# 619862306/CODON

Hardware: AMD Instinct MI355X
Metric: HR depth maps/sec (fwd) (higher is better)
Workload: dtype f32

## Files before the change

codon_amd/csrc/conv_wgrad_f32.hip:

```cpp

#include "codon_common.h"
#include "kernels.h"

namespace codon {

struct WgradParams {
  const float* x;
  const float* gy;
  float* ws;
  int H, W, cin, cout;
  long x_img, g_img, x_base, g_base;
  int tiles_x, band_tiles_y, nbands;
  int nsplit;
};

template <int KS, int CO_T, int CI_T>
__global__ __launch_bounds__(256, 2) void conv_wgrad_f32_kernel(const WgradParams p) {
  constexpr int PAD = KS / 2;
  constexpr int TW = 32, TH = 4;
  constexpr int XR = TH + KS - 1, XQ = TW + KS - 1;
  constexpr int XPL = (XR * XQ) | 1;
  constexpr int GPL = (TH * TW) | 1;
  constexpr int NCI = CI_T * 32, NCO = CO_T * 32;
  constexpr int XS = NCI * XPL, GS = NCO * GPL;
  constexpr int TAPS = KS * KS;
  constexpr int NT = CO_T * CI_T * TAPS;
  constexpr int TPW = (NT + 3) / 4;
  constexpr int XE = (NCI * XR * XQ + 255) / 256;
  constexpr int GE = (NCO * TH * TW) / 256;

  __shared__ float lds[XS + GS];
  float* const xs = lds;
  float* const gs = lds + XS;

  const int tid = threadIdx.x, lane = tid & 63, wave = tid >> 6;
  const int l31 = lane & 31, half = lane >> 5;
  const int H = p.H, W = p.W;
  const long HW = (long)H * W;

  const int nci_t = p.cin / NCI;
  const int cot = blockIdx.x / nci_t, cit = blockIdx.x % nci_t;
  const int split = blockIdx.y;
  const int b = split / p.nbands, band = split % p.nbands;
  const int ty_begin = band * p.band_tiles_y;
  const int tiles_y = (H + TH - 1) / TH;
  const int ty_end = min(ty_begin + p.band_tiles_y, tiles_y);

  const float* __restrict__ xg = p.x + b * p.x_img + p.x_base + (long)cit * NCI * HW;
  const float* __restrict__ gg = p.gy + b * p.g_img + p.g_base + (long)cot * NCO * HW;

  int a_off[TPW], b_off[TPW];
#pragma unroll
  for (int j = 0; j < TPW; ++j) {
    int t = wave + 4 * j;
    if (t >= NT) t = NT - 1;
    const int tap = t % TAPS;
    const int cc = t / TAPS;
    const int ci_t = cc % CI_T, co_t = cc / CI_T;
    const int dy = tap / KS, dx = tap % KS;
    a_off[j] = (co_t * 32 + l31) * GPL + half;
    b_off[j] = (ci_t * 32 + l31) * XPL + dy * XQ + dx + half;
  }

  f32x16 acc[TPW];
#pragma unroll
  for (int j = 0; j < TPW; ++j)
#pragma unroll
    for (int r = 0; r < 16; ++r) acc[j][r] = 0.f;

#pragma unroll 1
  for (int ty = ty_begin; ty < ty_end; ++ty) {
#pragma unroll 1
    for (int tx = 0; tx < p.tiles_x; ++tx) {
      const int tx0 = tx * TW, ty0 = ty * TH;
      __syncthreads();
#pragma unroll 6
      for (int k = 0; k < XE; ++k) {
        const int e = tid + k * 256;
        const int c = e / (XR * XQ);
        const int rem = e - c * (XR * XQ);
        const int r = rem / XQ, q = rem - r * XQ;
        const int gy_ = ty0 + r - PAD, gx_ = tx0 + q - PAD;
        if (e < NCI * XR * XQ) {
          const bool ok = gy_ >= 0 && gy_ < H && gx_ >= 0 && gx_ < W;
          const float v = xg[ok ? c * HW + (long)gy_ * W + gx_ : 0];
          xs[c * XPL + rem] = ok ? v : 0.f;
        }
      }
#pragma unroll 8
      for (int k = 0; k < GE; ++k) {
        const int e = tid + k * 256;
        const int c = e / (TH * TW);
        const int rem = e - c * (TH * TW);
        const int r = rem / TW, q = rem - r * TW;
        const int gy_ = ty0 + r, gx_ = tx0 + q;
        const bool ok = gy_ < H && gx_ < W;
        const float v = gg[ok ? c * HW + (long)gy_ * W + gx_ : 0];
        gs[c * GPL + rem] = ok ? v : 0.f;
      }
      __syncthreads();
#pragma unroll 1
      for (int r = 0; r < TH; ++r) {
#pragma unroll 4
        for (int q = 0; q < TW; q += 2) {
          const int po = r * TW + q, xo = r * XQ + q;
#pragma unroll
          for (int j = 0; j < TPW; ++j) {
            const float a = gs[a_off[j] + po];
            const float bv = xs[b_off[j] + xo];
            acc[j] = __builtin_amdgcn_mfma_f32_32x32x2f32(a, bv, acc[j], 0, 0, 0);
          }
        }
      }
    }
  }

  float* __restrict__ wsp = p.ws + (long)split * TAPS * p.cout * p.cin;
#pragma unroll
  for (int j = 0; j < TPW; ++j) {
    const int t = wave + 4 * j;
    if (t < NT) {
      const int tap = t % TAPS;
      const int cc = t / TAPS;
      const int ci_t = cc % CI_T, co_t = cc / CI_T;
      const int ci = cit * NCI + ci_t * 32 + l31;
#pragma unroll
      for (int r = 0; r < 16; ++r) {
        const int co = cot * NCO + co_t * 32 + (r & 3) + 8 * (r >> 2) + 4 * half;
        wsp[((long)tap * p.cout + co) * p.cin + ci] = acc[j][r];
      }
    }
  }
}

__global__ __launch_bounds__(256) void wgrad_reduce_kernel(const float* __restrict__ ws, float* __restrict__ dw,
                                                           int cout, int cin, int taps, int nsplit, int accumulate) {
  const long n = (long)cout * cin * taps;
  const long i = (blockIdx.x * 256L + threadIdx.x) * 4;
  if (i >= n) return;
  const int ci = (int)(i % cin);
  const long t = i / cin;
  const int co = (int)(t % cout);
  const int tap = (int)(t / cout);
  float4 s = make_float4(0.f, 0.f, 0.f, 0.f);
  int k = 0;
  for (; k + 8 <= nsplit; k += 8) {
    float4 v[8];
#pragma unroll
    for (int j = 0; j < 8; ++j) v[j] = *reinterpret_cast<const float4*>(ws + (long)(k + j) * n + i);
#pragma unroll
    for (int j = 0; j < 8; ++j) { s.x += v[j].x; s.y += v[j].y; s.z += v[j].z; s.w += v[j].w; }
  }
  for (; k < nsplit; ++k) {
    const float4 v = *reinterpret_cast<const float4*>(ws + (long)k * n + i);
    s.x += v.x; s.y += v.y; s.z += v.z; s.w += v.w;
  }
  float* o = dw + ((long)co * cin + ci) * taps + tap;
  const float r[4] = {s.x, s.y, s.z, s.w};
#pragma unroll
  for (int j = 0; j < 4; ++j) o[(long)j * taps] = accumulate ? o[(long)j * taps] + r[j] : r[j];
}

int launch_wgrad_reduce(const float* ws, float* dw, int cout, int cin, int taps, int nsplit, int accumulate,
                        hipStream_t stream) {
  const long n = (long)cout * cin * taps;
  if (cin % 4 != 0 || ((uintptr_t)ws % 16) != 0) {
    set_error("wgrad_reduce: cin %d not a multiple of 4 or workspace not 16-byte aligned", cin);
    return CODON_ERR_BAD_ARG;
  }
  hipLaunchKernelGGL(wgrad_reduce_kernel, dim3((unsigned)((n / 4 + 255) / 256)), dim3(256), 0, stream, ws, dw, cout, cin,
                     taps, nsplit, accumulate);
  return check_launch("wgrad_reduce_kernel");
}

struct WgradPlan {
  int co_t, ci_t, nbands, band_tiles_y, nsplit, nchan_blocks;
  bool t16;
};

static bool wgrad_plan(const codon_conv_desc* d, WgradPlan* pl) {
  const int k = d->ksize, ci = d->cin, co = d->cout;
  if (k == 5 && ((ci == 128 && co == 128) || (ci == 64 && co == 64))) { pl->co_t = 1; pl->ci_t = 1; }
  else if (k == 3 && ((ci == 64 || ci == 128) && co == 64)) { pl->co_t = 2; pl->ci_t = 1; }
  else if (k == 1 && ci == 128 && co == 64) { pl->co_t = 2; pl->ci_t = 2; }
  else return false;
  pl->nchan_blocks = (co / (32 * pl->co_t)) * (ci / (32 * pl->ci_t));
  pl->t16 = conv_wgrad_f32_t16_shape(d);
  const int plan_blocks = pl->t16 ? (co / 64) * (ci / (k == 1 ? 128 : 32)) : pl->nchan_blocks;
  const int target = pl->t16 ? 256 : 1024;
  const int tiles_y = (d->height + 3) / 4;
  const int want = wgrad_band_count(target, plan_blocks, d->batch, tiles_y);
  pl->band_tiles_y = (tiles_y + want - 1) / want;
  pl->nbands = (tiles_y + pl->band_tiles_y - 1) / pl->band_tiles_y;
  pl->nsplit = d->batch * pl->nbands;
  return true;
}

size_t conv_wgrad_workspace_bytes(const codon_conv_desc* d) {
  WgradPlan pl;
  if (!wgrad_plan(d, &pl)) return 0;
  return (size_t)pl.nsplit * d->cout * d->cin * d->ksize * d->ksize * sizeof(float);
}

template <int KS, int CO_T, int CI_T>
static void launch_wgrad(const WgradParams& p, int nchan_blocks, hipStream_t stream) {
  hipLaunchKernelGGL((conv_wgrad_f32_kernel<KS, CO_T, CI_T>), dim3(nchan_blocks, p.nsplit), dim3(256), 0, stream, p);
}

int conv2d_wgrad_f32(const codon_conv_desc* d, const float* x, const float* gy, float* dw, float* workspace,
                     size_t ws_bytes, int accumulate, hipStream_t stream) {
  WgradPlan pl;
  if (!wgrad_plan(d, &pl)) {
    set_error("conv2d_wgrad: no f32 kernel for k=%d cin=%d cout=%d", d->ksize, d->cin, d->cout);
    return CODON_ERR_UNSUPPORTED;
  }
  CODON_REQUIRE(ws_bytes >= conv_wgrad_workspace_bytes(d), CODON_ERR_BAD_ARG,
                "conv2d_wgrad: workspace %zu B < required %zu B", ws_bytes, conv_wgrad_workspace_bytes(d));
  CODON_REQUIRE(pl.nsplit <= 65535, CODON_ERR_UNSUPPORTED, "conv2d_wgrad: %d splits > 65535", pl.nsplit);
  if (pl.t16 && conv_wgrad_f32_t16_supported(d, x, gy)) {
    const int st = launch_wgrad_f32_t16(d, x, gy, workspace, pl.nbands, pl.nsplit, stream);
    if (st != CODON_OK || accumulate == CODON_WGRAD_DEFER) return st;
    return launch_wgrad_reduce(workspace, dw, d->cout, d->cin, d->ksize * d->ksize, pl.nsplit, accumulate, stream);
  }
  WgradParams p = wgrad_fill<WgradParams>(d, x, gy, workspace, 1, pl.nbands, pl.nsplit);
  p.band_tiles_y = pl.band_tiles_y;
  if (d->ksize == 5) launch_wgrad<5, 1, 1>(p, pl.nchan_blocks, stream);
  else if (d->ksize == 3) launch_wgrad<3, 2, 1>(p, pl.nchan_blocks, stream);
  else launch_wgrad<1, 2, 2>(p, pl.nchan_blocks, stream);
  int st = check_launch("conv_wgrad_f32_kernel");
  if (st != CODON_OK || accumulate == CODON_WGRAD_DEFER) return st;
  return launch_wgrad_reduce(workspace, dw, d->cout, d->cin, d->ksize * d->ksize, pl.nsplit, accumulate, stream);
}

}
```

codon_amd/csrc/conv_wgrad_f32_t16.hip:

```cpp

#include <type_traits>

#include "codon_common.h"
#include "kernels.h"

namespace codon {

typedef unsigned t16_u32x4 __attribute__((ext_vector_type(4)));
typedef unsigned t16_u32x2 __attribute__((ext_vector_type(2)));

typedef const volatile __attribute__((address_space(3))) float* lds_rf;

template <int N, class F, int I = 0>
__device__ __forceinline__ void t16_static_for(F&& f) {
  if constexpr (I < N) {
    f(std::integral_constant<int, I>{});
    t16_static_for<N, F, I + 1>(static_cast<F&&>(f));
  }
}

struct WgradT16Params {
  const float* x;
  const float* gy;
  float* ws;
  int H, W, cin, cout;
  long x_img, g_img, x_base, g_base;
  int tiles_x, nbands, nsplit;
};

template <int KS>
__global__ __launch_bounds__(512, 2) void conv_wgrad_f32_t16_kernel(const WgradT16Params p) {
  constexpr int PAD = KS / 2, TAPS = KS * KS;
  constexpr int NCIT = KS == 1 ? 4 : 1;
  constexpr int NCI = 32 * NCIT;
  constexpr int NACC = TAPS * NCIT;
  constexpr int TW = 32, TH = KS == 1 ? 2 : 4;
  constexpr int XL = KS == 1 ? 0 : 4;
  constexpr int XC = TW + 2 * XL, XR = TH + KS - 1;
  constexpr int XPL = ((XR * XC + 29) / 32) * 32 + 2;
  constexpr int GPL = TH * TW + 2;
  static_assert(XPL >= XR * XC && XPL % 32 == 2 && GPL % 32 == 2, "plane strides");
  constexpr int XW = NCI * XPL, GW = 64 * GPL;
  constexpr int NXC = NCI * XR * (XC / 4), NGC = 64 * TH * (TW / 4);
  constexpr int NT = 512;
  constexpr int XE = (NXC + NT - 1) / NT, GE = NGC / NT;
  static_assert(NGC % NT == 0, "gy tile is a whole number of staging rounds");
  constexpr unsigned OOB = 0xFFFFFFF0u;

  __shared__ __attribute__((aligned(16))) float lds[2 * (XW + GW)];

  const int tid = threadIdx.x, lane = tid & 63, wave = tid >> 6;
  const int l15 = lane & 15, kq = lane >> 4;
  const int H = p.H, W = p.W;
  const long HW = (long)H * W;
  const unsigned HW4 = 4u * (unsigned)H * (unsigned)W;

  const int nci_b = p.cin / NCI;
  const unsigned vb_ = xcd_remap(blockIdx.y * gridDim.x + blockIdx.x, gridDim.x * gridDim.y);
  const int bx_ = (int)(vb_ % gridDim.x), by_ = (int)(vb_ / gridDim.x);
  const int cob = bx_ / nci_b, cib = bx_ % nci_b;
  const int split = by_;
  const int b = split / p.nbands, band = split % p.nbands;
  const int tiles_y = (H + TH - 1) / TH;
  const int ty_begin = (int)((long)band * tiles_y / p.nbands);
  const int ty_end = (int)((long)(band + 1) * tiles_y / p.nbands);
  const int ntile = (ty_end - ty_begin) * p.tiles_x;

  const float* const xg = p.x + b * p.x_img + p.x_base + (long)cib * NCI * HW;
  const float* const gg = p.gy + b * p.g_img + p.g_base + (long)cob * 64 * HW;

  unsigned xrel[XE], grel[GE];
  int xrc[XE], grc[GE];
  int xlds[XE], glds[GE];
#pragma unroll
  for (int k = 0; k < XE; ++k) {
    const int e = tid + k * NT;
    const int ch = e % (XC / 4), r = (e / (XC / 4)) % XR, c = e / ((XC / 4) * XR);
    const bool in = (NXC % NT == 0) || e < NXC;
    xrel[k] = (unsigned)c * HW4 + 4u * (unsigned)(r * W + ch * 4);
    xrc[k] = in ? ((r << 8) | ch) : -1;
    xlds[k] = in ? c * XPL + r * XC + ch * 4 : 0;
  }
#pragma unroll
  for (int k = 0; k < GE; ++k) {
    const int e = tid + k * NT;
    const int ch = e % (TW / 4), r = (e / (TW / 4)) % TH, c = e / ((TW / 4) * TH);
    grel[k] = (unsigned)c * HW4 + 4u * (unsigned)(r * W + ch * 4);
    grc[k] = (r << 8) | ch;
    glds[k] = c * GPL + r * TW + ch * 4;
  }

  const int co16 = wave & 3, ci16 = wave >> 2;
  const int a_lane = (co16 * 16 + l15) * GPL + kq;
  const int b_lane = (ci16 * 16 * NCIT + l15) * XPL + kq + (XL - PAD);

  f32x4 acc[NACC];
#pragma unroll
  for (int j = 0; j < NACC; ++j)
#pragma unroll
    for (int r = 0; r < 4; ++r) acc[j][r] = 0.f;

  t16_u32x4 xv[XE], gv[GE];
  auto load_tile = [&](int t) {
    const int ty = ty_begin + t / p.tiles_x, tx = t % p.tiles_x;
    const int tx0 = tx * TW, ty0 = ty * TH;
    const __amdgpu_buffer_rsrc_t xr = __builtin_amdgcn_make_buffer_rsrc(
        (void*)(xg + ((long)(ty0 - PAD) * W + (tx0 - XL))), 0, (int)OOB, 0x00020000);
    const __amdgpu_buffer_rsrc_t gr = __builtin_amdgcn_make_buffer_rsrc(
        (void*)(gg + ((long)ty0 * W + tx0)), 0, (int)OOB, 0x00020000);
#pragma unroll
    for (int k = 0; k < XE; ++k) {
      const int gy_ = ty0 - PAD + (xrc[k] >> 8), gx_ = tx0 - XL + 4 * (xrc[k] & 255);
      const bool ok = xrc[k] >= 0 && gy_ >= 0 && gy_ < H && gx_ >= 0 && gx_ < W;
      const auto v = __builtin_amdgcn_raw_buffer_load_b128(xr, ok ? xrel[k] : OOB, 0, 0);
      xv[k] = *reinterpret_cast<const t16_u32x4*>(&v);
    }
#pragma unroll
    for (int k = 0; k < GE; ++k) {
      const int gy_ = ty0 + (grc[k] >> 8), gx_ = tx0 + 4 * (grc[k] & 255);
      const bool ok = gy_ < H && gx_ < W;
      const auto v = __builtin_amdgcn_raw_buffer_load_b128(gr, ok ? grel[k] : OOB, 0, 0);
      gv[k] = *reinterpret_cast<const t16_u32x4*>(&v);
    }
  };
  auto store_tile = [&](int buf) {
    float* xs = lds + buf * (XW + GW);
    float* gs = xs + XW;
#pragma unroll
    for (int k = 0; k < XE; ++k)
      if ((NXC % NT == 0) || tid + k * NT < NXC) {
        *reinterpret_cast<t16_u32x2*>(xs + xlds[k]) = t16_u32x2{xv[k][0], xv[k][1]};
        *reinterpret_cast<t16_u32x2*>(xs + xlds[k] + 2) = t16_u32x2{xv[k][2], xv[k][3]};
      }
#pragma unroll
    for (int k = 0; k < GE; ++k) {
      *reinterpret_cast<t16_u32x2*>(gs + glds[k]) = t16_u32x2{gv[k][0], gv[k][1]};
      *reinterpret_cast<t16_u32x2*>(gs + glds[k] + 2) = t16_u32x2{gv[k][2], gv[k][3]};
    }
  };

  if (ntile > 0) {
    load_tile(0);
    store_tile(0);
  }
  __syncthreads();

#pragma unroll 1
  for (int t = 0; t < ntile; ++t) {
    const bool has_next = t + 1 < ntile;
    if (has_next) load_tile(t + 1);

    const float* xs = lds + (t & 1) * (XW + GW);
    const float* gs = xs + XW;
    const lds_rf ap = (lds_rf)(gs + a_lane);
    const lds_rf bp = (lds_rf)(xs + b_lane);
    float a[2], bv[2][NACC];
#define T16_FETCH(set_, r_, q_)                                                           \
    {                                                                                     \
      a[set_] = ap[(r_) * TW + (q_)];                                                     \
      _Pragma("unroll") for (int ct = 0; ct < NCIT; ++ct)                                 \
        _Pragma("unroll") for (int dy = 0; dy < KS; ++dy)                                 \
          _Pragma("unroll") for (int dx = 0; dx < KS; ++dx)                               \
            bv[set_][ct * TAPS + dy * KS + dx] = bp[ct * 16 * XPL + ((r_) + dy) * XC + (q_) + dx]; \
    }
    T16_FETCH(0, 0, 0)
    t16_static_for<TH * (TW / 4)>([&](auto sc) {
      constexpr int s_ = decltype(sc)::value;
      constexpr int cur = s_ & 1;
      if constexpr (s_ + 1 < TH * (TW / 4)) T16_FETCH(cur ^ 1, (s_ + 1) / (TW / 4), ((s_ + 1) % (TW / 4)) * 4)
      __builtin_amdgcn_sched_barrier(0);
#pragma unroll
      for (int j = 0; j < NACC; ++j) acc[j] = __builtin_amdgcn_mfma_f32_16x16x4f32(a[cur], bv[cur][j], acc[j], 0, 0, 0);
      __builtin_amdgcn_sched_barrier(0);
    });
#undef T16_FETCH
    if (has_next) store_tile((t + 1) & 1);
    __syncthreads();
  }

  float* __restrict__ wsp = p.ws + (long)split * TAPS * p.cout * p.cin;
#pragma unroll
  for (int ct = 0; ct < NCIT; ++ct) {
    const int ci = cib * NCI + (ci16 * NCIT + ct) * 16 + l15;
#pragma unroll
    for (int tap = 0; tap < TAPS; ++tap)
#pragma unroll
      for (int r = 0; r < 4; ++r) {
        const int co = cob * 64 + co16 * 16 + 4 * kq + r;
        wsp[((long)tap * p.cout + co) * p.cin + ci] = acc[ct * TAPS + tap][r];
      }
  }
}

bool conv_wgrad_f32_t16_shape(const codon_conv_desc* d) {
  if (d->ksize == 1 && d->cin % 128 != 0) return false;
  return (d->ksize == 1 || d->ksize == 3 || d->ksize == 5) && d->width % 4 == 0 && d->cout % 64 == 0 && d->cin % 32 == 0 &&
         (long)d->height * d->width * 4 * 128 < 0xFFFFFFF0L;
}

bool conv_wgrad_f32_t16_supported(const codon_conv_desc* d, const void* x, const void* gy) {
  if (!conv_wgrad_f32_t16_shape(d)) return false;
  const long HW = (long)d->height * d->width;
  const uintptr_t xa = reinterpret_cast<uintptr_t>(x) + 4 * (uintptr_t)(d->x_coff * HW);
  const uintptr_t ga = reinterpret_cast<uintptr_t>(gy) + 4 * (uintptr_t)(d->y_coff * HW);
  return (xa % 16) == 0 && (ga % 16) == 0 && ((d->x_ctotal * HW * 4) % 16) == 0 && ((d->y_ctotal * HW * 4) % 16) == 0;
}

int launch_wgrad_f32_t16(const codon_conv_desc* d, const float* x, const float* gy, float* workspace, int nbands,
                         int nsplit, hipStream_t stream) {
  const WgradT16Params p = wgrad_fill<WgradT16Params>(d, x, gy, workspace, 1, nbands, nsplit);
  const dim3 grid((d->cout / 64) * (d->cin / (d->ksize == 1 ? 128 : 32)), nsplit);
  if (d->ksize == 5) hipLaunchKernelGGL(conv_wgrad_f32_t16_kernel<5>, grid, dim3(512), 0, stream, p);
  else if (d->ksize == 3) hipLaunchKernelGGL(conv_wgrad_f32_t16_kernel<3>, grid, dim3(512), 0, stream, p);
  else hipLaunchKernelGGL(conv_wgrad_f32_t16_kernel<1>, grid, dim3(512), 0, stream, p);
  return check_launch("conv_wgrad_f32_t16_kernel");
}

}
```

Measured before the change: 32.27.

## Stage wgrad tiles with direct buffer-to-LDS loads interleaved into MFMA loop

Replaces the register-staged global load + LDS store of the next x/gy tile with per-dword buffer_load ... lds instructions. Their issue is spread across the first half of the MFMA K-loop, so copying the next tile overlaps compute without holding it in VGPRs. It adds an interior-tile fast path that skips per-element bounds checks and uses per-plane buffer resources. It also drops the width%4 and 16-byte alignment requirements, widening the t16 path to more shapes, but k=1 with unaligned width is routed back to the old kernel. The tradeoff is narrower 4-byte loads instead of 128-bit loads, plus a waitcnt/barrier at each tile end.

After: 32.21. About the same (-0.2%).

```diff
diff --git a/codon_amd/csrc/conv_wgrad_f32.hip b/codon_amd/csrc/conv_wgrad_f32.hip
--- a/codon_amd/csrc/conv_wgrad_f32.hip
+++ b/codon_amd/csrc/conv_wgrad_f32.hip
@@ -186,8 +186,9 @@
   else return false;
   pl->nchan_blocks = (co / (32 * pl->co_t)) * (ci / (32 * pl->ci_t));
   pl->t16 = conv_wgrad_f32_t16_shape(d);
-  const int plan_blocks = pl->t16 ? (co / 64) * (ci / (k == 1 ? 128 : 32)) : pl->nchan_blocks;
-  const int target = pl->t16 ? 256 : 1024;
+  const bool plan_t16 = pl->t16 && d->width % 4 == 0;
+  const int plan_blocks = plan_t16 ? (co / 64) * (ci / (k == 1 ? 128 : 32)) : pl->nchan_blocks;
+  const int target = plan_t16 ? 256 : 1024;
   const int tiles_y = (d->height + 3) / 4;
   const int want = wgrad_band_count(target, plan_blocks, d->batch, tiles_y);
   pl->band_tiles_y = (tiles_y + want - 1) / want;
@@ -217,7 +218,8 @@
   CODON_REQUIRE(ws_bytes >= conv_wgrad_workspace_bytes(d), CODON_ERR_BAD_ARG,
                 "conv2d_wgrad: workspace %zu B < required %zu B", ws_bytes, conv_wgrad_workspace_bytes(d));
   CODON_REQUIRE(pl.nsplit <= 65535, CODON_ERR_UNSUPPORTED, "conv2d_wgrad: %d splits > 65535", pl.nsplit);
-  if (pl.t16 && conv_wgrad_f32_t16_supported(d, x, gy)) {
+  const bool k1_recorded = d->ksize == 1 && d->width % 4 != 0;
+  if (pl.t16 && !k1_recorded && conv_wgrad_f32_t16_supported(d, x, gy)) {
     const int st = launch_wgrad_f32_t16(d, x, gy, workspace, pl.nbands, pl.nsplit, stream);
     if (st != CODON_OK || accumulate == CODON_WGRAD_DEFER) return st;
     return launch_wgrad_reduce(workspace, dw, d->cout, d->cin, d->ksize * d->ksize, pl.nsplit, accumulate, stream);
diff --git a/codon_amd/csrc/conv_wgrad_f32_t16.hip b/codon_amd/csrc/conv_wgrad_f32_t16.hip
--- a/codon_amd/csrc/conv_wgrad_f32_t16.hip
+++ b/codon_amd/csrc/conv_wgrad_f32_t16.hip
@@ -41,15 +41,24 @@
   constexpr int GPL = TH * TW + 2;
   static_assert(XPL >= XR * XC && XPL % 32 == 2 && GPL % 32 == 2, "plane strides");
   constexpr int XW = NCI * XPL, GW = 64 * GPL;
-  constexpr int NXC = NCI * XR * (XC / 4), NGC = 64 * TH * (TW / 4);
-  constexpr int NT = 512;
-  constexpr int XE = (NXC + NT - 1) / NT, GE = NGC / NT;
-  static_assert(NGC % NT == 0, "gy tile is a whole number of staging rounds");
+  constexpr int NWV = 8;
+  constexpr int XPLANE = XR * XC, GPLANE = TH * TW;
+  constexpr int XJ = (XPLANE + 63) / 64, GJ = GPLANE / 64;
+  static_assert(GPLANE % 64 == 0 && XJ * 64 <= XPL && GJ * 64 <= GPL, "a piece stays inside its padded plane");
+  constexpr int XPW = NCI / NWV, GPW = 64 / NWV;
+  static_assert(NCI % NWV == 0, "x planes are dealt evenly over the waves");
+  constexpr int NPX = XPW * XJ, NPIECE = NPX + GPW * GJ;
+  constexpr int NSTEP = TH * (TW / 4);
+  constexpr int PPS = KS == 1 ? 8 : 2;
+  static_assert(PPS * (NSTEP / 2 + 2) >= NPIECE, "the tile's pieces are all issued by the middle of the K loop");
   constexpr unsigned OOB = 0xFFFFFFF0u;
+  constexpr int RSRC_FLAGS = 0x00020000;
+  typedef __attribute__((address_space(3))) void lds_void;
 
   __shared__ __attribute__((aligned(16))) float lds[2 * (XW + GW)];
 
-  const int tid = threadIdx.x, lane = tid & 63, wave = tid >> 6;
+  const int tid = threadIdx.x, lane = tid & 63;
+  const int wave = __builtin_amdgcn_readfirstlane(tid >> 6);
   const int l15 = lane & 15, kq = lane >> 4;
   const int H = p.H, W = p.W;
   const long HW = (long)H * W;
@@ -68,26 +77,22 @@
 
   const float* const xg = p.x + b * p.x_img + p.x_base + (long)cib * NCI * HW;
   const float* const gg = p.gy + b * p.g_img + p.g_base + (long)cob * 64 * HW;
-
-  unsigned xrel[XE], grel[GE];
-  int xrc[XE], grc[GE];
-  int xlds[XE], glds[GE];
-#pragma unroll
-  for (int k = 0; k < XE; ++k) {
-    const int e = tid + k * NT;
-    const int ch = e % (XC / 4), r = (e / (XC / 4)) % XR, c = e / ((XC / 4) * XR);
-    const bool in = (NXC % NT == 0) || e < NXC;
-    xrel[k] = (unsigned)c * HW4 + 4u * (unsigned)(r * W + ch * 4);
-    xrc[k] = in ? ((r << 8) | ch) : -1;
-    xlds[k] = in ? c * XPL + r * XC + ch * 4 : 0;
-  }
-#pragma unroll
-  for (int k = 0; k < GE; ++k) {
-    const int e = tid + k * NT;
-    const int ch = e % (TW / 4), r = (e / (TW / 4)) % TH, c = e / ((TW / 4) * TH);
-    grel[k] = (unsigned)c * HW4 + 4u * (unsigned)(r * W + ch * 4);
-    grc[k] = (r << 8) | ch;
-    glds[k] = c * GPL + r * TW + ch * 4;
+  const __amdgpu_buffer_rsrc_t xr = __builtin_amdgcn_make_buffer_rsrc((void*)xg, 0, (int)((unsigned)NCI * HW4), RSRC_FLAGS);
+  const __amdgpu_buffer_rsrc_t gr = __builtin_amdgcn_make_buffer_rsrc((void*)gg, 0, (int)(64u * HW4), RSRC_FLAGS);
+
+  unsigned xrel[XJ], grel[GJ];
+  int xrc[XJ], grc[GJ];
+#pragma unroll
+  for (int j = 0; j < XJ; ++j) {
+    const int w = j * 64 + lane, r = w / XC, q = w - r * XC;
+    xrel[j] = 4u * (unsigned)(r * W + q);
+    xrc[j] = (XPLANE % 64 == 0 || w < XPLANE) ? ((r << 8) | q) : -1;
+  }
+#pragma unroll
+  for (int j = 0; j < GJ; ++j) {
+    const int w = j * 64 + lane, r = w / TW, q = w - r * TW;
+    grel[j] = 4u * (unsigned)(r * W + q);
+    grc[j] = (r << 8) | q;
   }
 
   const int co16 = wave & 3, ci16 = wave >> 2;
@@ -100,55 +105,62 @@
 #pragma unroll
     for (int r = 0; r < 4; ++r) acc[j][r] = 0.f;
 
-  t16_u32x4 xv[XE], gv[GE];
-  auto load_tile = [&](int t) {
+  unsigned xvo[XJ], gvo[GJ];
+  auto plan_tile = [&](int t) {
     const int ty = ty_begin + t / p.tiles_x, tx = t % p.tiles_x;
     const int tx0 = tx * TW, ty0 = ty * TH;
-    const __amdgpu_buffer_rsrc_t xr = __builtin_amdgcn_make_buffer_rsrc(
-        (void*)(xg + ((long)(ty0 - PAD) * W + (tx0 - XL))), 0, (int)OOB, 0x00020000);
-    const __amdgpu_buffer_rsrc_t gr = __builtin_amdgcn_make_buffer_rsrc(
-        (void*)(gg + ((long)ty0 * W + tx0)), 0, (int)OOB, 0x00020000);
-#pragma unroll
-    for (int k = 0; k < XE; ++k) {
-      const int gy_ = ty0 - PAD + (xrc[k] >> 8), gx_ = tx0 - XL + 4 * (xrc[k] & 255);
-      const bool ok = xrc[k] >= 0 && gy_ >= 0 && gy_ < H && gx_ >= 0 && gx_ < W;
-      const auto v = __builtin_amdgcn_raw_buffer_load_b128(xr, ok ? xrel[k] : OOB, 0, 0);
-      xv[k] = *reinterpret_cast<const t16_u32x4*>(&v);
-    }
-#pragma unroll
-    for (int k = 0; k < GE; ++k) {
-      const int gy_ = ty0 + (grc[k] >> 8), gx_ = tx0 + 4 * (grc[k] & 255);
-      const bool ok = gy_ < H && gx_ < W;
-      const auto v = __builtin_amdgcn_raw_buffer_load_b128(gr, ok ? grel[k] : OOB, 0, 0);
-      gv[k] = *reinterpret_cast<const t16_u32x4*>(&v);
+    const unsigned xorg = 4u * (unsigned)((ty0 - PAD) * W + (tx0 - XL));
+    const unsigned gorg = 4u * (unsigned)(ty0 * W + tx0);
+    const bool interior = ty0 >= PAD && ty0 + TH + PAD <= H && tx0 >= XL && tx0 - XL + XC <= W;
+    if (interior) {
+#pragma unroll
+      for (int j = 0; j < XJ; ++j) xvo[j] = xrc[j] >= 0 ? xorg + xrel[j] : OOB;
+#pragma unroll
+      for (int j = 0; j < GJ; ++j) gvo[j] = gorg + grel[j];
+    } else {
+#pragma unroll
+      for (int j = 0; j < XJ; ++j) {
+        const int gy_ = ty0 - PAD + (xrc[j] >> 8), gx_ = tx0 - XL + (xrc[j] & 255);
+        const bool ok = xrc[j] >= 0 && gy_ >= 0 && gy_ < H && gx_ >= 0 && gx_ < W;
+        xvo[j] = ok ? xorg + xrel[j] : OOB;
+      }
+#pragma unroll
+      for (int j = 0; j < GJ; ++j) {
+        const int gy_ = ty0 + (grc[j] >> 8), gx_ = tx0 + (grc[j] & 255);
+        gvo[j] = (gy_ < H && gx_ < W) ? gorg + grel[j] : OOB;
+      }
     }
   };
-  auto store_tile = [&](int buf) {
-    float* xs = lds + buf * (XW + GW);
-    float* gs = xs + XW;
-#pragma unroll
-    for (int k = 0; k < XE; ++k)
-      if ((NXC % NT == 0) || tid + k * NT < NXC) {
-        *reinterpret_cast<t16_u32x2*>(xs + xlds[k]) = t16_u32x2{xv[k][0], xv[k][1]};
-        *reinterpret_cast<t16_u32x2*>(xs + xlds[k] + 2) = t16_u32x2{xv[k][2], xv[k][3]};
-      }
-#pragma unroll
-    for (int k = 0; k < GE; ++k) {
-      *reinterpret_cast<t16_u32x2*>(gs + glds[k]) = t16_u32x2{gv[k][0], gv[k][1]};
-      *reinterpret_cast<t16_u32x2*>(gs + glds[k] + 2) = t16_u32x2{gv[k][2], gv[k][3]};
+  auto issue_piece = [&](auto ic, float* buf) {
+    constexpr int i = decltype(ic)::value;
+    if constexpr (i < NPX) {
+      constexpr int c = i / XJ, j = i % XJ;
+      const int plane = wave * XPW + c;
+      __builtin_amdgcn_raw_ptr_buffer_load_lds(xr, (lds_void*)(buf + plane * XPL + j * 64), 4, xvo[j], (unsigned)plane * HW4, 0, 0);
+    } else if constexpr (i < NPIECE) {
+      constexpr int c = (i - NPX) / GJ, j = (i - NPX) % GJ;
+      const int plane = wave * GPW + c;
+      __builtin_amdgcn_raw_ptr_buffer_load_lds(gr, (lds_void*)(buf + XW + plane * GPL + j * 64), 4, gvo[j], (unsigned)plane * HW4, 0, 0);
     }
   };
 
   if (ntile > 0) {
-    load_tile(0);
-    store_tile(0);
-  }
+    plan_tile(0);
+    t16_static_for<NPIECE>([&](auto ic) { issue_piece(ic, lds); });
+  }
+  __builtin_amdgcn_s_waitcnt(0x0070);
   __syncthreads();
 
 #pragma unroll 1
   for (int t = 0; t < ntile; ++t) {
-    const bool has_next = t + 1 < ntile;
-    if (has_next) load_tile(t + 1);
+    if (t + 1 < ntile) plan_tile(t + 1);
+    else {
+#pragma unroll
+      for (int j = 0; j < XJ; ++j) xvo[j] = OOB;
+#pragma unroll
+      for (int j = 0; j < GJ; ++j) gvo[j] = OOB;
+    }
+    float* const nbuf = lds + ((t + 1) & 1) * (XW + GW);
 
     const float* xs = lds + (t & 1) * (XW + GW);
     const float* gs = xs + XW;
@@ -164,17 +176,25 @@
             bv[set_][ct * TAPS + dy * KS + dx] = bp[ct * 16 * XPL + ((r_) + dy) * XC + (q_) + dx]; \
     }
     T16_FETCH(0, 0, 0)
-    t16_static_for<TH * (TW / 4)>([&](auto sc) {
+    t16_static_for<NSTEP>([&](auto sc) {
       constexpr int s_ = decltype(sc)::value;
       constexpr int cur = s_ & 1;
-      if constexpr (s_ + 1 < TH * (TW / 4)) T16_FETCH(cur ^ 1, (s_ + 1) / (TW / 4), ((s_ + 1) % (TW / 4)) * 4)
+      if constexpr (s_ + 1 < NSTEP) T16_FETCH(cur ^ 1, (s_ + 1) / (TW / 4), ((s_ + 1) % (TW / 4)) * 4)
       __builtin_amdgcn_sched_barrier(0);
-#pragma unroll
-      for (int j = 0; j < NACC; ++j) acc[j] = __builtin_amdgcn_mfma_f32_16x16x4f32(a[cur], bv[cur][j], acc[j], 0, 0, 0);
+      constexpr int HALF = NACC / 2;
+#pragma unroll
+      for (int j = 0; j < HALF; ++j) acc[j] = __builtin_amdgcn_mfma_f32_16x16x4f32(a[cur], bv[cur][j], acc[j], 0, 0, 0);
+      if constexpr (s_ * PPS < NPIECE) {
+        __builtin_amdgcn_sched_barrier(0);
+        t16_static_for<PPS>([&](auto kc) { issue_piece(std::integral_constant<int, s_ * PPS + decltype(kc)::value>{}, nbuf); });
+        __builtin_amdgcn_sched_barrier(0);
+      }
+#pragma unroll
+      for (int j = HALF; j < NACC; ++j) acc[j] = __builtin_amdgcn_mfma_f32_16x16x4f32(a[cur], bv[cur][j], acc[j], 0, 0, 0);
       __builtin_amdgcn_sched_barrier(0);
     });
 #undef T16_FETCH
-    if (has_next) store_tile((t + 1) & 1);
+    __builtin_amdgcn_s_waitcnt(0x0070);
     __syncthreads();
   }
 
@@ -194,16 +214,12 @@
 
 bool conv_wgrad_f32_t16_shape(const codon_conv_desc* d) {
   if (d->ksize == 1 && d->cin % 128 != 0) return false;
-  return (d->ksize == 1 || d->ksize == 3 || d->ksize == 5) && d->width % 4 == 0 && d->cout % 64 == 0 && d->cin % 32 == 0 &&
+  return (d->ksize == 1 || d->ksize == 3 || d->ksize == 5) && d->cout % 64 == 0 && d->cin % 32 == 0 &&
          (long)d->height * d->width * 4 * 128 < 0xFFFFFFF0L;
 }
 
 bool conv_wgrad_f32_t16_supported(const codon_conv_desc* d, const void* x, const void* gy) {
-  if (!conv_wgrad_f32_t16_shape(d)) return false;
-  const long HW = (long)d->height * d->width;
-  const uintptr_t xa = reinterpret_cast<uintptr_t>(x) + 4 * (uintptr_t)(d->x_coff * HW);
-  const uintptr_t ga = reinterpret_cast<uintptr_t>(gy) + 4 * (uintptr_t)(d->y_coff * HW);
-  return (xa % 16) == 0 && (ga % 16) == 0 && ((d->x_ctotal * HW * 4) % 16) == 0 && ((d->y_ctotal * HW * 4) % 16) == 0;
+  return conv_wgrad_f32_t16_shape(d) && reinterpret_cast<uintptr_t>(x) % 4 == 0 && reinterpret_cast<uintptr_t>(gy) % 4 == 0;
 }
 
 int launch_wgrad_f32_t16(const codon_conv_desc* d, const float* x, const float* gy, float* workspace, int nbands,
```
